# Diegotistical/OptionsLab

Hardware: AMD Instinct MI355X
Metric: MC path-steps/sec (1M paths × 252 steps Euro call); price vs BS |err|/σ (higher is better)
Workload: dtype f32 normals / f64 prices

## Files before the change

include/olmc.h:

```cpp
#ifndef OLMC_H
#define OLMC_H

#include <stdint.h>

#ifdef __cplusplus
extern "C" {
#endif

#define OLMC_ABI_VERSION 6

enum {
    OLMC_OK = 0,
    OLMC_ERR_ARG = 1,
    OLMC_ERR_HIP = 2,
    OLMC_ERR_STATE = 3,
    OLMC_ERR_RCCL = 4
};

enum { OLMC_STREAM_GBM = 0, OLMC_STREAM_HESTON = 1, OLMC_STREAM_JUMP = 2, OLMC_STREAM_KOU = 3 };
enum { OLMC_STREAM_HESTON_QE = 0x48514500 };
enum { OLMC_AVG_ARITHMETIC = 0, OLMC_AVG_GEOMETRIC = 1, OLMC_AVG_ARITHMETIC_FAST = 2 };
#define OLMC_MAX_BATCH 16

typedef struct olmc_stats {
// ... 269 lines not shown
                               int n_gpus, olmc_cv_moments* out);
int olmc_multi_gpu_european_qmc(double S, double K, double T, double r, double sigma, double q, int is_call,
                                int64_t n_paths, int32_t dims, const uint32_t* sv, const uint32_t* shift, int32_t bits,
                                int n_gpus, olmc_stats* out);
int olmc_multi_gpu_european_qmc_greeks_fd(double S, double K, double T, double r, double sigma, double q, int is_call,
                                          int64_t n_paths, int32_t dims, const uint32_t* sv, const uint32_t* shift, int32_t bits,
                                          int second_order, int n_gpus, double* out9, olmc_stats* evals );
int olmc_multi_gpu_european_qmc_cv(double S, double K, double T, double r, double sigma, double q, int is_call,
                                   int64_t n_paths, int32_t dims, const uint32_t* sv, const uint32_t* shift, int32_t bits,
                                   int n_gpus, olmc_cv_moments* out);
int olmc_multi_gpu_spans(double* out8);

int olmc_fetch_dev(const double* d_src, int32_t n, void* hip_stream, double* out_host);

int olmc_combine_stats(const olmc_stats* parts, int32_t n_parts, double r, double T, olmc_stats* out);

int olmc_philox_words(uint64_t seed, int64_t path_offset, int64_t n_paths,
                      int32_t block0, int32_t n_blocks, uint32_t stream_tag, uint32_t* out_host);
int olmc_normals(uint64_t seed, int64_t path_offset, int64_t n_paths, int32_t n_steps,
                 float* out_host);

int olmc_profile_enable(int on);
enum { OLMC_TUNE_GRID_CAP = 2, OLMC_TUNE_QMC_BLOCK = 4, OLMC_TUNE_SPLIT_TAIL = 7, OLMC_TUNE_POLL = 8, OLMC_TUNE_SPLIT_SAT = 9,
       OLMC_TUNE_MULTI_LAUNCH = 10, OLMC_TUNE_STAGED_COPY = 11, OLMC_TUNE_PHILOX_TABLE = 12 };
int olmc_tune(int knob, int value);
int olmc_profile_reset(void);
int olmc_kernel_time(int64_t* launches, double* total_ms);

#ifdef __cplusplus
}
#endif
#endif
```

include/olmc_probe.h:

```cpp
#ifndef OLMC_PROBE_H
#define OLMC_PROBE_H
#include "olmc.h"

#ifdef __cplusplus
extern "C" {
#endif

int olmc_exp2_probe(const double* x_host, int64_t n, double* y_host);
int olmc_exp2_probe_form(const double* x_host, int64_t n, double* y_host, int form);
int olmc_ndtri_probe(const double* p_host, int64_t n, double* z_host, int form);
int olmc_box_muller_probe(const uint32_t* xa, const uint32_t* xb, int64_t n, float* z_cos, float* z_sin, float* pair);
int olmc_sqrt_nonneg_probe(const double* x, int64_t n, double* y);
int olmc_normal_moments(uint64_t seed, int64_t path_offset, int64_t n_paths, int32_t n_steps, double* out4);
int olmc_reduce_probe(int nv, int form, int values, int blocking, int32_t launches, const int64_t* n_threads, const uint64_t* salt,
                      double* out);
int olmc_rows_sum_probe(int nv, int whole_workgroup, const double* rows_host, int32_t rows, double* out_nv);
int olmc_wave_reduce_probe(int p, int op, const double* v_host, double* out);

int olmc_phase_stamps(int64_t n_paths, int32_t n_steps, uint64_t seed, int32_t lead_launches, uint64_t* stamps_host, int64_t capacity,
                      int64_t* info3);

int olmc_clock_probe(int64_t n_paths, int32_t n_steps, uint64_t seed, double* out3);

enum { OLMC_PROBE_MAD_U64_U32 = 0, OLMC_PROBE_BITOP3_B32, OLMC_PROBE_CVT_F32_U32, OLMC_PROBE_FMAMK_F32, OLMC_PROBE_AND_OR_B32,
       OLMC_PROBE_LOG_F32, OLMC_PROBE_SQRT_F32, OLMC_PROBE_SIN_F32, OLMC_PROBE_COS_F32, OLMC_PROBE_EXP_F32, OLMC_PROBE_ADD_F32,
       OLMC_PROBE_FMA_F32, OLMC_PROBE_CVT_F64_F32, OLMC_PROBE_ADD_F64, OLMC_PROBE_FMA_F64, OLMC_PROBE_RNDNE_F64,
       OLMC_PROBE_LDEXP_F64, OLMC_PROBE_CVT_I32_F64,
       OLMC_PROBE_MIX_LOG_ADD, OLMC_PROBE_MIX_LOG_BITOP3, OLMC_PROBE_BITOP3_VVV, OLMC_PROBE_BITOP3_VVC, OLMC_PROBE_XOR_VV,
       OLMC_PROBE_MIX_BITOP3_ADD, OLMC_PROBE_MIX_MAD_BITOP3, OLMC_PROBE_MAD_U64_U32_VV, OLMC_PROBE_COUNT };
int olmc_issue_probe(int op, int waves_per_simd, double* ns_per_instr);

int olmc_european_f64_normals(double S, double K, double T, double r, double sigma, double q, int is_call, int64_t n_paths,
                              int32_t n_steps, uint64_t seed, olmc_stats* out);

int olmc_launch_gap_probe(int32_t n, double* us_per_launch);

enum { OLMC_PROBE_TUNE_FAULT_SHARD = 5, OLMC_PROBE_TUNE_FORCE_NV = 6, OLMC_PROBE_TUNE_MULTI_REHEARSAL = 11, OLMC_PROBE_TUNE_EXPECT_TABLE = 12 };
int olmc_probe_tune(int knob, int value);

#ifdef __cplusplus
}
#endif
#endif
```

optionslab_amd/_hip.py:

```python
from __future__ import annotations

import ctypes as C
import importlib.util
import os
import sys
import threading
from typing import List, Optional, Sequence, Tuple

import numpy as np

from .exceptions import AccelerationError

LIBRARY_PATH = os.environ.get("OLMC_LIBRARY") or os.path.join(os.path.dirname(os.path.abspath(__file__)), "libolmc.so")
MAX_BATCH = 16
AVG_ARITHMETIC, AVG_GEOMETRIC, AVG_ARITHMETIC_FAST = 0, 1, 2
_U64 = (1 << 64) - 1


class Stats(C.Structure):
    _fields_ = [("sum", C.c_double), ("sumsq", C.c_double), ("n", C.c_int64),
                ("price", C.c_double), ("std_error", C.c_double)]


class Option(C.Structure):
# ... 964 lines not shown


def philox_words(seed: int, path_offset: int, n_paths: int, block0: int, n_blocks: int, tag: int = 0) -> np.ndarray:
    out = np.empty((int(n_paths), int(n_blocks), 4), dtype=np.uint32)
    _check(lib().olmc_philox_words(seed64(seed), int(path_offset), int(n_paths), int(block0), int(n_blocks), int(tag),
                                   _pointer(out, C.c_uint32)))
    return out


def normals(seed: int, path_offset: int, n_paths: int, n_steps: int) -> np.ndarray:
    out = np.empty((int(n_paths), int(n_steps)), dtype=np.float32)
    _check(lib().olmc_normals(seed64(seed), int(path_offset), int(n_paths), int(n_steps), _pointer(out, C.c_float)))
    return out


TUNE_GRID_CAP = 2
TUNE_QMC_BLOCK = 4
TUNE_SPLIT_TAIL = 7
TUNE_POLL = 8
TUNE_SPLIT_SAT = 9
TUNE_MULTI_LAUNCH = 10
TUNE_STAGED_COPY = 11
TUNE_PHILOX_TABLE = 12


def tune(knob: int, value: int) -> None:
    _check(load_library().olmc_tune(int(knob), int(value)))


def profile_enable(on: bool) -> None:
    _check(lib().olmc_profile_enable(int(on)))


def profile_reset() -> None:
    _check(lib().olmc_profile_reset())


def kernel_time() -> Tuple[int, float]:
    n, ms = C.c_int64(0), C.c_double(0.0)
    _check(lib().olmc_kernel_time(C.byref(n), C.byref(ms)))
    return n.value, ms.value
```

optionslab_amd/csrc/olmc.hip:

```cpp
#include "olmc.h"
#include "olmc_local_vol.h"
#include "olmc_local_vol_qmc.h"
#include "olmc_jump.h"
#include "olmc_kernels.h"
#include "olmc_local_vol_kernels.h"
#include "olmc_local_vol_qmc_kernels.h"
#include "olmc_jump_kernels.h"
#include "olmc_jump_scenario_kernels.h"
#include "olmc_job_board.h"
#include "olmc_device_mem.h"

#include <dlfcn.h>
#include <sched.h>
#include <time.h>
#include <hip/hip_ext.h>
#include <rccl/rccl.h>

#include <algorithm>
#include <atomic>
#include <chrono>
#include <climits>
#include <condition_variable>
#include <cmath>
#include <cstdio>
// ... 47 lines not shown
    int device = -1;
    int cus = 0;
    hipStream_t stream = nullptr;
    struct WsSlot {
        DeviceBlock<Mem> block_rows;
        DeviceBlock<Mem> group_rows;
        DeviceBlock<Mem> counters;
        hipEvent_t done = nullptr;
        bool used = false;
        bool claimed = false;
        hipStream_t owner = nullptr;
        bool shared = false;
    };
    static constexpr int kSlots = 8;
    WsSlot slots[kSlots + 1];
    int next_slot = 0, cur_slot = 0;
    uint64_t* h_flag = nullptr;
    uint64_t* d_flag = nullptr;
    uint64_t seq = 0;
    uint64_t armed = 0;
    PinnedBlock<Mem> result;
    double* h_result = nullptr;
    double* d_result = nullptr;
    DeviceBlock<Mem> bulk;
    PinnedBlock<Mem> stage[2];
    hipEvent_t stage_landed[2] = {nullptr, nullptr};
    BatchWorkspace<Mem, MultiOption, kMultiCounterStride> multi;
    CachedUpload<Mem> sobol;
    CachedUpload<Mem> bridge;
    DeviceBlock<Mem> heston_w;
    CachedUpload<Mem> lv;
    int drain() const { return Mem::wait(stream); }
    bool busy = false;
    std::vector<EventPair> ev_free, ev_pending;
    int64_t prof_launches = 0;
    double prof_ms = 0.0;
};

constexpr int kMaxContexts = 8;

struct DevicePool {
    std::mutex mu;
    std::condition_variable idle;
    std::vector<DeviceCtx*> all;
    int device = -1;
};
// ... 1 lines not shown
std::mutex g_mu;
std::atomic<DevicePool*> g_pool[kMaxDevices] = {};
std::atomic<int> g_default_device{-1};
bool g_profile = false;

int no_users() { return 0; }

int ctx_allocate(DeviceCtx* c) {
    HIP_TRY(hipStreamCreateWithFlags(&c->stream, hipStreamNonBlocking));
    for (auto& sl : c->slots) {
        int rc = sl.group_rows.reserve(sizeof(double) * kMaxNV * kMaxGroups, no_users);
        if (!rc) rc = sl.counters.reserve(kCounterBytes, no_users);
        if (rc) return rc;
        HIP_TRY(hipMemset(sl.counters.get(), 0, kCounterBytes));
        HIP_TRY(hipEventCreateWithFlags(&sl.done, hipEventDisableTiming));
    }
    const int rc = c->result.reserve(sizeof(double) * (kMaxNV + 1 + 15), no_users, 0, 0, true);
    if (rc) return rc;
    c->h_result = c->result.as<double>();
    c->d_result = c->result.alias<double>();
    c->h_flag = reinterpret_cast<uint64_t*>(c->h_result + kMaxNV + 8);
    c->d_flag = reinterpret_cast<uint64_t*>(c->d_result + kMaxNV + 8);
    *c->h_flag = 0;
    return OLMC_OK;
}

void ctx_release(DeviceCtx* c) {
    if (c->stream) (void)hipStreamSynchronize(c->stream);
    for (auto& ep : c->ev_pending) { (void)hipEventDestroy(ep.start); (void)hipEventDestroy(ep.stop); }
    for (auto& ep : c->ev_free) { (void)hipEventDestroy(ep.start); (void)hipEventDestroy(ep.stop); }
    for (hipEvent_t ev : c->stage_landed)
        if (ev) (void)hipEventDestroy(ev);
    for (auto& sl : c->slots)
        if (sl.done) (void)hipEventDestroy(sl.done);
    if (c->stream) (void)hipStreamDestroy(c->stream);
    delete c;
}

int ctx_create(int device, DeviceCtx** out) {
    int count = 0;
    hipError_t e = hipGetDeviceCount(&count);
    if (e != hipSuccess || count <= 0)
        return fail(OLMC_ERR_HIP, std::string("no HIP device available: ") + hipGetErrorString(e));
    if (device < 0 || device >= count || device >= kMaxDevices)
        return fail(OLMC_ERR_ARG, "device index out of range");
    HIP_TRY(hipSetDevice(device));
// ... 12 lines not shown
}

struct CtxLease {
    DeviceCtx* c = nullptr;
    DevicePool* pool = nullptr;
    CtxLease() = default;
    CtxLease(const CtxLease&) = delete;
    CtxLease& operator=(const CtxLease&) = delete;
    ~CtxLease() { release(); }
    void release() {
        if (!c) return;
        {
            std::lock_guard<std::mutex> lock(pool->mu);
            c->busy = false;
        }
        pool->idle.notify_all();
        c = nullptr;
    }
};

int ctx_lease_on(int dev, CtxLease* out) {
    DevicePool* pool = g_pool[dev].load(std::memory_order_acquire);
    if (!pool) return fail(OLMC_ERR_STATE, "device not initialised (call olmc_init)");
    HIP_TRY(hipSetDevice(dev));
    std::unique_lock<std::mutex> lock(pool->mu);
    for (;;) {
        for (DeviceCtx* c : pool->all)
            if (!c->busy) {
                c->busy = true;
                out->c = c;
                out->pool = pool;
                return OLMC_OK;
            }
        if (static_cast<int>(pool->all.size()) < kMaxContexts) {
            DeviceCtx* c = nullptr;
            const int rc = ctx_create(dev, &c);
            if (rc) return rc;
            c->busy = true;
            pool->all.push_back(c);
            out->c = c;
            out->pool = pool;
            return OLMC_OK;
        }
        pool->idle.wait(lock);
    }
}

// ... 91 lines not shown
    }
    if (err == hipSuccess) landed.store(n_chunks, std::memory_order_release);
    else give_up.store(true);
    const auto t_join = clock::now();
    for (std::thread& t : threads) t.join();
    if (trace)
        std::fprintf(stderr, "[olmc copy_to_host] %.1f MB, %lld chunks, %d threads: spawn %.0f us, first chunk landed (kernel + DMA) %.0f us, later event waits %.0f us, "
                             "waits for the copy threads %.0f us, last chunk out + join %.0f us, total %.0f us\n", bytes / 1e6, static_cast<long long>(n_chunks), n_threads,
                     us_spawn, us_first, us_events, us_workers, us_since(t_join), us_since(t_begin));
    if (err != hipSuccess) {
        (void)hipStreamSynchronize(c->stream);
        (void)hipGetLastError();
        return fail(OLMC_ERR_HIP, std::string("copy_to_host: ") + hipGetErrorString(err));
    }
    return OLMC_OK;
}

int g_multi_launch = 0;
int g_grid_cap = 0;
int g_qmc_block = 0;
int g_poll = 0;
int g_split_tail = 0;
int g_philox_table = 1;
int g_split_sat = 0;
#ifdef OLMC_WITH_PROBES
int g_fault_shard = 0;
int g_force_nv = 0;
int g_multi_rehearsal = 0;
int g_expect_table = 0;
std::atomic<int> g_expect_table_misses{0};
#endif

int32_t grid_for(int64_t n_paths, int32_t n_steps = INT32_MAX) { return path_grid(n_paths, n_steps, g_grid_cap); }

template <typename Kernel>
int resident_workgroups(Kernel kernel) {
    static std::mutex mu;
    static std::vector<std::pair<const void*, int>> cache;
    const void* key = reinterpret_cast<const void*>(kernel);
    std::lock_guard<std::mutex> lock(mu);
    for (const auto& e : cache)
        if (e.first == key) return e.second;
    int nb = 0;
    if (hipOccupancyMaxActiveBlocksPerMultiprocessor(&nb, kernel, kBlock, 0) != hipSuccess || nb < 1) {
        (void)hipGetLastError();
        nb = 1;
    }
    cache.emplace_back(key, nb);
    return nb;
}

int32_t european_launch_shape(const DeviceCtx* c, PathRange* pr, int occ, bool keep_grid = false) {
// ... 3 lines not shown
    const int64_t wgs = (pr->count + kBlock - 1) / kBlock;
    if (g_split_tail < 0 || grid_cap != 0 || wgs != grid) return grid;
    if ((pr->n_steps >> 2) / kGroup < 4 || c->cus < 1) return grid;
    int64_t per_cu = (pr->count / kBlock) / c->cus;
    if (occ >= 1 && g_split_sat > 0) {
        const int64_t r = per_cu % occ;
        if (r > 0 && r < std::min(g_split_sat, occ)) per_cu -= r;
    }
    const int64_t full = per_cu * c->cus;
    const int64_t rest = pr->count - full * kBlock;
    if (rest == 0) return grid;
    const int64_t split = (rest + kWave - 1) / kWave;
    if (full + split > kMaxGrid) return grid;
    pr->split_from = static_cast<int32_t>(full);
    return static_cast<int32_t>(full + split);
}

template <int NSETS, int MODE>
int european_occupancy(bool anti) {
    if (g_split_sat <= 0) return 0;
    return anti ? resident_workgroups(european_path_kernel<NSETS, true, MODE, false>) : resident_workgroups(european_path_kernel<NSETS, false, MODE, false>);
}

int make_ws(DeviceCtx* c, hipStream_t stream, int32_t grid, int nv, double* d_out, double tail, ReduceWs* ws) {
    const bool own = stream == c->stream;
    int idx = DeviceCtx::kSlots;
    if (!own) {
        idx = -1;
        for (int i = 0; i < DeviceCtx::kSlots && idx < 0; ++i)
            if (c->slots[i].claimed && !c->slots[i].shared && c->slots[i].owner == stream) idx = i;
        for (int i = 0; i < DeviceCtx::kSlots && idx < 0; ++i)
            if (!c->slots[i].claimed) { c->slots[i].claimed = true; c->slots[i].owner = stream; idx = i; }
        if (idx < 0) {
            idx = c->next_slot;
            c->next_slot = (c->next_slot + 1) % DeviceCtx::kSlots;
            DeviceCtx::WsSlot& taken = c->slots[idx];
            if (!taken.shared) {
                HIP_TRY(hipDeviceSynchronize());
                taken.shared = true;
                taken.used = false;
            }
        }
    }
    DeviceCtx::WsSlot& sl = c->slots[idx];
    c->cur_slot = idx;
    const bool guarded = !own && sl.shared;
    const size_t need = static_cast<size_t>(grid) * nv;
    int rc = sl.block_rows.reserve(sizeof(double) * need, [&] {
        if (!guarded) HIP_TRY(hipStreamSynchronize(stream));
        else if (sl.used) HIP_TRY(hipEventSynchronize(sl.done));
        return static_cast<int>(OLMC_OK);
    }, sizeof(double) << 16);
    if (rc) return rc;
    if (guarded && sl.used) HIP_TRY(hipStreamWaitEvent(stream, sl.done, 0));
    ws->block_rows = sl.block_rows.as<double>();
    ws->group_rows = sl.group_rows.as<double>();
    ws->counters = sl.counters.as<uint32_t>();
    ws->out = d_out;
    ws->tail = tail;
    ws->row_capacity = sl.block_rows.capacity() / sizeof(double);
#ifdef OLMC_WITH_PROBES
    if (g_force_nv > 0) ws->row_capacity = static_cast<uint64_t>(grid) * g_force_nv;
#endif
    ws->done_flag = nullptr;
    ws->done_value = 0;
    c->armed = 0;
    if (own && d_out == c->d_result && g_poll >= 0) {
        c->armed = ++c->seq;
        ws->done_flag = c->d_flag;
        ws->done_value = c->armed;
    }
    return OLMC_OK;
}

void ws_recover(DeviceCtx* c) {
    c->armed = 0;
    (void)hipDeviceSynchronize();
    (void)hipGetLastError();
    for (auto& sl : c->slots) (void)hipMemset(sl.counters.get(), 0, kCounterBytes);
}

void multi_recover(DeviceCtx* c) {
    c->armed = 0;
    (void)hipDeviceSynchronize();
    (void)hipGetLastError();
    if (c->multi.counters()) (void)hipMemset(c->multi.counters(), 0, c->multi.counter_bytes());
}

int after_launch(DeviceCtx* c, hipStream_t stream) {
    hipError_t e = hipGetLastError();
    if (e != hipSuccess) { ws_recover(c); return fail(OLMC_ERR_HIP, std::string("kernel launch: ") + hipGetErrorString(e)); }
    if (c->cur_slot == DeviceCtx::kSlots || !c->slots[c->cur_slot].shared) return OLMC_OK;
    DeviceCtx::WsSlot& sl = c->slots[c->cur_slot];
    HIP_TRY(hipEventRecord(sl.done, stream));
    sl.used = true;
    return OLMC_OK;
}

int prof_begin(DeviceCtx* c, hipStream_t s, EventPair* ep) {
    if (c->ev_free.empty()) {
        HIP_TRY(hipEventCreate(&ep->start));
        HIP_TRY(hipEventCreate(&ep->stop));
    } else {
        *ep = c->ev_free.back();
        c->ev_free.pop_back();
    }
// ... 172 lines not shown
            launch_european<1, kReduce>(anti, g, st, pr, cs, ws, nullptr, timed);
        } else if (nsets == 8) {
            fused(std::integral_constant<int, 8>{});
        } else {
            fused(std::integral_constant<int, 16>{});
        }
    }, profiled);
}

constexpr int64_t kSpinUs = 200, kYieldUs = 2000, kSleepUs = 20;

struct TimerSlack {
    long old = -1;
    void tighten() {
        if (old >= 0) return;
        old = prctl(PR_GET_TIMERSLACK, 0, 0, 0, 0);
        if (old >= 0 && prctl(PR_SET_TIMERSLACK, 1000UL, 0, 0, 0) != 0) old = -1;
    }
    ~TimerSlack() {
        if (old >= 0) (void)prctl(PR_SET_TIMERSLACK, static_cast<unsigned long>(old), 0, 0, 0);
    }
};

int wait_armed(DeviceCtx* c, hipStream_t s) {
    if (c->armed != 0) {
        const uint64_t want = c->armed;
        c->armed = 0;
        using clock = std::chrono::steady_clock;
        const auto t0 = clock::now();
        bool queried = false;
        int phase = 0;
        TimerSlack slack;
        for (uint32_t spins = 0;; ++spins) {
            if (__atomic_load_n(c->h_flag, __ATOMIC_ACQUIRE) == want) {
                if (queried) (void)hipGetLastError();
                return OLMC_OK;
            }
            if (phase == 0) {
                __builtin_ia32_pause();
                if ((spins & 0x3F) == 0x3F && clock::now() - t0 >= std::chrono::microseconds(kSpinUs)) phase = 1;
                continue;
            }
            if (phase == 1) {
                sched_yield();
                if ((spins & 0xF) == 0xF && clock::now() - t0 >= std::chrono::microseconds(kYieldUs)) phase = 2;
                continue;
            }
            if ((spins & 0x3F) == 0) {
                const hipError_t q = hipStreamQuery(s);
                queried = true;
                if (q == hipSuccess) break;
                if (q != hipErrorNotReady) {
                    ws_recover(c);
                    return fail(OLMC_ERR_HIP, std::string("hipStreamQuery: ") + hipGetErrorString(q));
                }
            }
            slack.tighten();
            const timespec nap{0, kSleepUs * 1000};
            nanosleep(&nap, nullptr);
        }
        (void)hipGetLastError();
    }
    hipError_t e = hipStreamSynchronize(s);
    if (e != hipSuccess) { ws_recover(c); return fail(OLMC_ERR_HIP, std::string("hipStreamSynchronize: ") + hipGetErrorString(e)); }
    return OLMC_OK;
}

int sync_or_recover(DeviceCtx* c, hipStream_t s) {
    if (s != c->stream) c->armed = 0;
    return wait_armed(c, s);
}

int run_batch(const olmc_option* opts, int32_t k, int64_t path_offset, int64_t n_local, int32_t n_steps,
              uint64_t seed, int antithetic, olmc_stats* out, bool prices_only = false, bool keep_grid = false) {
    if (!opts || !out) return fail(OLMC_ERR_ARG, "null pointer");
    if (k < 1 || k > OLMC_MAX_BATCH) return fail(OLMC_ERR_ARG, "batch size must be in [1, OLMC_MAX_BATCH]");
    int rc = check_paths(path_offset, n_local, n_steps);
    if (rc) return rc;
    CtxLease lease;
    rc = ctx_lease(&lease);
    if (rc) return rc;
    DeviceCtx* const c = lease.c;
    int pos[OLMC_MAX_BATCH];
    bool lean = prices_only;
    rc = run_batch_device(c, c->stream, opts, k, path_offset, n_local, n_steps, seed, antithetic, c->d_result, -1.0, pos, true, &lean, keep_grid);
    if (rc) return rc;
    finish_set(c->h_result, pos, n_local * (antithetic ? 2 : 1), opts, k, false, lean, out);
    return OLMC_OK;
}

}

// ... 91 lines not shown
                                       int64_t path_offset, int64_t n_local, int32_t n_steps, uint64_t seed,
                                       int antithetic, double* d_triple, void* hip_stream) {
    if (!d_triple) return fail(OLMC_ERR_ARG, "null pointer");
    int rc = check_paths(path_offset, n_local, n_steps);
    if (rc) return rc;
    CtxLease lease;
    rc = ctx_lease(&lease);
    if (rc) return rc;
    DeviceCtx* const c = lease.c;
    hipStream_t s = static_cast<hipStream_t>(hip_stream);
    const olmc_option o = make_option(S, K, T, r, sigma, q, is_call);
    const double n = static_cast<double>(n_local * (antithetic ? 2 : 1));
    return run_batch_device(c, s, &o, 1, path_offset, n_local, n_steps, seed, antithetic, d_triple, n, nullptr, true);
}

namespace {
int fetch_dev(DeviceCtx* c, const double* d_src, int32_t n, hipStream_t s, double* out_host) {
    const uint64_t want = ++c->seq;
    hipLaunchKernelGGL(publish_kernel, dim3(1), dim3(kWave), 0, s, d_src, n, c->d_result, c->d_flag, want);
    HIP_TRY(hipGetLastError());
    int rc = OLMC_OK;
    if (g_poll >= 0) {
        c->armed = want;
        rc = wait_armed(c, s);
    } else {
        hipError_t e = hipStreamSynchronize(s);
        if (e != hipSuccess) rc = fail(OLMC_ERR_HIP, std::string("hipStreamSynchronize: ") + hipGetErrorString(e));
    }
    if (rc) return rc;
    for (int32_t i = 0; i < n; ++i) out_host[i] = c->h_result[i];
    return OLMC_OK;
}
}

extern "C" int olmc_fetch_dev(const double* d_src, int32_t n, void* hip_stream, double* out_host) {
    if (!d_src || !out_host) return fail(OLMC_ERR_ARG, "null pointer");
    if (n < 1 || n > kMaxNV + 1) return fail(OLMC_ERR_ARG, "n must be in [1, 33]");
    CtxLease lease;
    int rc = ctx_lease(&lease);
    if (rc) return rc;
    return fetch_dev(lease.c, d_src, n, static_cast<hipStream_t>(hip_stream), out_host);
}

extern "C" int olmc_european_batch(const olmc_option* opts, int32_t k, int64_t path_offset, int64_t n_local,
                                   int32_t n_steps, uint64_t seed, int antithetic, olmc_stats* out) {
    return run_batch(opts, k, path_offset, n_local, n_steps, seed, antithetic, out);
// ... 14 lines not shown
    if (rc) return rc;
    CtxLease lease;
    rc = ctx_lease(&lease);
    if (rc) return rc;
    DeviceCtx* const c = lease.c;
    const int32_t bpo = static_cast<int32_t>(std::min<int64_t>((n_paths + kBlock - 1) / kBlock, 1024));
    decltype(c->multi)::Views v;
    rc = c->multi.reserve(static_cast<size_t>(n_options), static_cast<size_t>(bpo), c->stream, &v);
    if (rc) return rc;
    MultiOption* const h = v.h_opts;
    for (int64_t j = 0; j < n_options; ++j) {
        const Contract ct = make_contract(opts[j], n_steps);
        h[j].a = ct.a; h[j].vol = ct.vol; h[j].strike = ct.strike; h[j].sign = ct.sign;
        h[j].tag = tags ? tags[j] : static_cast<uint32_t>(j);
        h[j].pad = 0;
    }
    HIP_TRY(hipMemcpyAsync(v.d_opts, h, sizeof(MultiOption) * n_options, hipMemcpyHostToDevice, c->stream));
    MultiDone md;
    md.done_count = v.d_done;
    md.n_total = static_cast<uint32_t>(n_options);
    md.done_flag = nullptr;
    md.done_value = 0;
    c->armed = 0;
    if (g_poll >= 0) {
        c->armed = ++c->seq;
        md.done_flag = c->d_flag;
        md.done_value = c->armed;
    }
    const PathRange pr = make_range(0, n_paths, n_steps, seed);
    EventPair ep{};
    if (g_profile) { rc = prof_begin(c, c->stream, &ep); if (rc) return rc; }
    for (int64_t base_opt = 0; base_opt < n_options; base_opt += 65535) {
        const unsigned ny = static_cast<unsigned>(std::min<int64_t>(65535, n_options - base_opt));
        with_bool(antithetic != 0, [&](auto a) { launch_timed(european_multi_kernel<a>, dim3(bpo, ny), dim3(kBlock), c->stream, nullptr, pr, v.d_opts, base_opt, v.d_rows, v.d_cnt, v.d_out, md); });
        hipError_t e = hipGetLastError();
        if (e != hipSuccess) {
            multi_recover(c);
            return fail(OLMC_ERR_HIP, std::string("kernel launch: ") + hipGetErrorString(e));
        }
    }
    if (g_profile) { rc = prof_end(c, c->stream, ep); if (rc) { multi_recover(c); return rc; } }
    rc = wait_armed(c, c->stream);
    if (rc) { multi_recover(c); return rc; }
    finish_set(v.h_out, nullptr, n_paths * (antithetic ? 2 : 1), opts, n_options, false, false, out);
    return OLMC_OK;
}
// ... 2745 lines not shown
    Carver bulk;
    rc = bulk_reserve(c, bytes, &bulk);
    if (rc) return rc;
    float* d_z = bulk.take<float>(bytes / sizeof(float));
    const int64_t total = n_paths * ((n_steps + 3) / 4);
    const int grid = static_cast<int>(std::min<int64_t>((total + 255) / 256, 4096));
    hipLaunchKernelGGL(normals_kernel, dim3(grid), dim3(256), 0, c->stream, static_cast<uint64_t>(path_offset), n_paths,
                       n_steps, static_cast<uint32_t>(seed), static_cast<uint32_t>(seed >> 32), d_z);
    HIP_TRY(hipGetLastError());
    HIP_TRY(hipMemcpyAsync(out_host, d_z, bytes, hipMemcpyDeviceToHost, c->stream));
    HIP_TRY(hipStreamSynchronize(c->stream));
    return OLMC_OK;
}

extern "C" int olmc_tune(int knob, int value) {
    if (knob == OLMC_TUNE_GRID_CAP && value >= 0) { g_grid_cap = value; return OLMC_OK; }
    if (knob == OLMC_TUNE_QMC_BLOCK && value >= -1 && value <= 2) { g_qmc_block = value; return OLMC_OK; }
    if (knob == OLMC_TUNE_POLL && value >= -1 && value <= 0) { g_poll = value; return OLMC_OK; }
    if (knob == OLMC_TUNE_SPLIT_TAIL && value >= -1 && value <= 0) { g_split_tail = value; return OLMC_OK; }
    if (knob == OLMC_TUNE_SPLIT_SAT && value >= 0 && value <= 16) { g_split_sat = value; return OLMC_OK; }
    if (knob == OLMC_TUNE_MULTI_LAUNCH && value >= -1 && value <= 0) { g_multi_launch = value; return OLMC_OK; }
    if (knob == OLMC_TUNE_STAGED_COPY && value >= -1 && value <= 0) { g_staged_copy = value; return OLMC_OK; }
    if (knob == OLMC_TUNE_PHILOX_TABLE && value >= 0 && value <= 1) { g_philox_table = value; return OLMC_OK; }
    return fail(OLMC_ERR_ARG, "unknown tuning knob or value");
}

namespace {
template <typename Fn>
int with_all_contexts(Fn fn) {
    int dev = t_device >= 0 ? t_device : g_default_device.load(std::memory_order_acquire);
    if (dev < 0) {
        int rc = olmc_init(0);
        if (rc) return rc;
        dev = t_device;
    }
    DevicePool* pool = g_pool[dev].load(std::memory_order_acquire);
    if (!pool) return fail(OLMC_ERR_STATE, "device not initialised (call olmc_init)");
    HIP_TRY(hipSetDevice(dev));
    std::vector<DeviceCtx*> mine;
    {
        std::unique_lock<std::mutex> lock(pool->mu);
        pool->idle.wait(lock, [&] { return std::none_of(pool->all.begin(), pool->all.end(), [](const DeviceCtx* c) { return c->busy; }); });
        mine = pool->all;
        for (DeviceCtx* c : mine) c->busy = true;
    }
    int rc = OLMC_OK;
// ... 56 lines not shown
```

optionslab_amd/csrc/olmc_host_math.h:

```cpp
#ifndef OLMC_HOST_MATH_H
#define OLMC_HOST_MATH_H

#include "olmc.h"
#include "olmc_jump_scenarios.h"

#include <algorithm>
#include <cmath>
#include <cstdint>
#include <cstring>

namespace olmc {

struct Contract {
    double a;
    double vol;
    double strike;
    double sign;
    double scale;
    double neg_sign_strike;
    double sign_scale;
};

template <int NSETS>
struct ContractSet {
// ... 581 lines not shown
    sh.blocks = qmc_block == 1 ? true : (qmc_block != 0 ? false : n_paths >= (int64_t(1) << blocks_from_log2));
    const int64_t split_grid = (n_paths + kWave - 1) / kWave;
    sh.split = !sh.blocks && (qmc_block == 0 || qmc_block == 2) && dims >= 16 && split_grid <= kMaxGrid;
    sh.units = sh.blocks ? (point_offset + n_paths + kQmcBlock - 1) / kQmcBlock - point_offset / kQmcBlock : n_paths;
    sh.grid = sh.split ? static_cast<int32_t>(split_grid) : path_grid(sh.units, INT32_MAX, grid_cap);
    return sh;
}

struct HestonSlabs {
    size_t slab;
    int32_t fit;
    int32_t grid;
    size_t bytes;
};
inline HestonSlabs heston_slab_shape(int32_t n_steps, int32_t grid, int cus, int32_t factors = 2) {
    HestonSlabs s;
    s.slab = static_cast<size_t>(factors) * static_cast<size_t>(n_steps) * kWave * sizeof(double);
    s.fit = static_cast<int32_t>(std::max<size_t>(kHestonSlabCap / (s.slab * kWavesPerBlock), 1));
    s.grid = std::min(grid, std::min(s.fit, std::max(cus, 1) * kHestonBridgeBlocksPerCu));
    s.bytes = s.slab * kWavesPerBlock * static_cast<size_t>(s.grid);
    return s;
}

}

#endif
```

optionslab_amd/csrc/olmc_kernels.h:

```cpp
#pragma once
#include <type_traits>
#include <hip/hip_runtime.h>
#include <stdint.h>

#include "olmc_host_math.h"

namespace olmc {



struct Words4 {
    uint32_t x0, x1, x2, x3;
};

__device__ __forceinline__ uint32_t xor3(uint32_t a, uint32_t b, uint32_t c) {
    return __builtin_amdgcn_bitop3_b32(a, b, c, 0x96);
}

__device__ __forceinline__ Words4 philox4x32_10(uint32_t c0, uint32_t c1, uint32_t c2, uint32_t c3,
                                                uint32_t k0, uint32_t k1) {
#pragma unroll
    for (int round = 0; round < 10; ++round) {
        const uint64_t p0 = static_cast<uint64_t>(kPhiloxM0) * c0;
        const uint64_t p1 = static_cast<uint64_t>(kPhiloxM1) * c2;
// ... 163 lines not shown
                                                  uint32_t tag = 0u) {
    return path_normal_quarters(g_lo, g_hi, n_steps, 0, 4, k0, k1, tag) * kPairZScale;
}

__device__ __forceinline__ double wave_sum(double v) {
#pragma unroll
    for (int off = kWave / 2; off > 0; off >>= 1) v += __shfl_down(v, off, kWave);
    return v;
}

constexpr int kGroupBlocks = 256;
constexpr int kGroupRowsCapacity = ((1 << 18) / kGroupBlocks + 1) * 32;
constexpr int kCounterStride = 64;

struct ReduceWs {
    double* block_rows;
    double* group_rows;
    uint32_t* counters;
    double* out;
    double tail;
    uint64_t row_capacity;
    uint64_t* done_flag;
    uint64_t done_value;
};

__device__ __forceinline__ void signal_done(const ReduceWs& ws) {
    if (ws.done_flag == nullptr) return;
    __builtin_amdgcn_fence(__ATOMIC_RELEASE, "");
    if (threadIdx.x == 0) __hip_atomic_store(ws.done_flag, ws.done_value, __ATOMIC_RELAXED, __HIP_MEMORY_SCOPE_SYSTEM);
}

#ifndef OLMC_AGENT_ACQUIRE
#define OLMC_AGENT_ACQUIRE 1
#endif
#if !OLMC_AGENT_ACQUIRE && defined(__HIP_DEVICE_COMPILE__) && !defined(__gfx942__) && !defined(__gfx950__)
#error "OLMC_AGENT_ACQUIRE=0 relies on gfx942 / gfx950 cache behaviour (sc1 rows are L2-served): build this target with the acquire"
#endif
__device__ __forceinline__ void acquire_rows() {
#if OLMC_AGENT_ACQUIRE
    __builtin_amdgcn_fence(__ATOMIC_ACQUIRE, "agent");
#else
    __builtin_amdgcn_fence(__ATOMIC_ACQUIRE, "wavefront");
#endif
}

__device__ __forceinline__ void store_sc1(double* p, double v) {
    __hip_atomic_store(p, v, __ATOMIC_RELAXED, __HIP_MEMORY_SCOPE_AGENT);
// ... 11 lines not shown
    double v = 0.0;
    if (c < NV) {
        constexpr int kBatch = 8;
        for (int32_t row = sub; row < rows; row += SUBS * kBatch) {
            double t[kBatch];
#pragma unroll
            for (int j = 0; j < kBatch; ++j) {
                const int32_t rj = row + j * SUBS;
                t[j] = rj < rows ? load_sc1(src + static_cast<size_t>(rj) * NV + c) : 0.0;
            }
#pragma unroll
            for (int j = 0; j < kBatch; ++j) v += t[j];
        }
    }
#pragma unroll
    for (int off = kWave / 2; off >= NVP; off >>= 1) v += __shfl_down(v, off, kWave);
    return v;
}

struct NoEpilogue {
    __device__ __forceinline__ void operator()(double) const {}
};

template <int NV, typename Epilogue = NoEpilogue>
__device__ __forceinline__ void grid_reduce(double v, const ReduceWs& ws, Epilogue done = Epilogue()) {
    const int lane = threadIdx.x;
    const int32_t n_blocks = static_cast<int32_t>(gridDim.x);
    const int32_t n_groups = (n_blocks + kGroupBlocks - 1) / kGroupBlocks;
    const int32_t group = static_cast<int32_t>(blockIdx.x) / kGroupBlocks;
    const int32_t group_size = min(kGroupBlocks, n_blocks - group * kGroupBlocks);

    if (static_cast<uint64_t>(n_blocks) * NV > ws.row_capacity || n_groups * NV > kGroupRowsCapacity) {
        if (blockIdx.x == 0) {
            if (lane < NV) ws.out[lane] = __builtin_nan("");
            signal_done(ws);
        }
        return;
    }
    if (lane < NV) store_sc1(ws.block_rows + static_cast<size_t>(blockIdx.x) * NV + lane, v);
    asm volatile("s_waitcnt vmcnt(0)" ::: "memory");
    uint32_t ticket = 0;
    if (lane == 0) ticket = __hip_atomic_fetch_add(ws.counters + static_cast<size_t>(group) * kCounterStride, 1u, __ATOMIC_RELAXED, __HIP_MEMORY_SCOPE_AGENT);
    ticket = __builtin_amdgcn_readfirstlane(ticket);
    if (ticket != static_cast<uint32_t>(group_size - 1)) return;

    acquire_rows();
    const double g = wave_rows_sum<NV>(ws.block_rows + static_cast<size_t>(group) * kGroupBlocks * NV, group_size);
    if (n_groups == 1) {
        if (lane < NV) ws.out[lane] = g;
        if (lane == 0) {
            if (ws.tail >= 0.0) ws.out[NV] = ws.tail;
            __hip_atomic_store(ws.counters, 0u, __ATOMIC_RELAXED, __HIP_MEMORY_SCOPE_AGENT);
        }
        done(g);
        signal_done(ws);
        return;
    }
    if (lane < NV) store_sc1(ws.group_rows + static_cast<size_t>(group) * NV + lane, g);
    asm volatile("s_waitcnt vmcnt(0)" ::: "memory");
    if (lane == 0) {
        __hip_atomic_store(ws.counters + static_cast<size_t>(group) * kCounterStride, 0u, __ATOMIC_RELAXED, __HIP_MEMORY_SCOPE_AGENT);
        ticket = __hip_atomic_fetch_add(ws.counters + static_cast<size_t>(n_groups) * kCounterStride, 1u, __ATOMIC_RELAXED, __HIP_MEMORY_SCOPE_AGENT);
    }
    ticket = __builtin_amdgcn_readfirstlane(ticket);
    if (ticket != static_cast<uint32_t>(n_groups - 1)) return;

    acquire_rows();
    const double total = wave_rows_sum<NV>(ws.group_rows, n_groups);
    if (lane < NV) ws.out[lane] = total;
    if (lane == 0) {
// ... 14 lines not shown
        constexpr int kBatch = NVP >= 16 ? 16 : 8;
        for (int32_t row = sub; row < rows; row += SUBS * kBatch) {
            double t[kBatch];
#pragma unroll
            for (int j = 0; j < kBatch; ++j) {
                const int32_t rj = row + j * SUBS;
                t[j] = rj < rows ? load_sc1(src + static_cast<size_t>(rj) * NV + c) : 0.0;
            }
#pragma unroll
            for (int j = 0; j < kBatch; ++j) v += t[j];
        }
    }
    part[threadIdx.x] = v;
    __syncthreads();
    double total = 0.0;
    if (threadIdx.x < NV) {
#pragma unroll
        for (int k = 0; k < SUBS; ++k) total += part[k * NVP + threadIdx.x];
    }
    __syncthreads();
    return total;
}

template <int NV, typename Epilogue = NoEpilogue>
__device__ __forceinline__ void grid_reduce_workgroup(double v, const ReduceWs& ws, Epilogue done = Epilogue()) {
    __shared__ double part[kBlock];
    __shared__ uint32_t last;
    const int t = threadIdx.x;
    const bool wave0 = t < kWave;
    const int32_t n_blocks = static_cast<int32_t>(gridDim.x);
    const int32_t n_groups = (n_blocks + kGroupBlocks - 1) / kGroupBlocks;
    const int32_t group = static_cast<int32_t>(blockIdx.x) / kGroupBlocks;
    const int32_t group_size = min(kGroupBlocks, n_blocks - group * kGroupBlocks);

    if (static_cast<uint64_t>(n_blocks) * NV > ws.row_capacity || n_groups * NV > kGroupRowsCapacity) {
        if (blockIdx.x == 0 && wave0) {
            if (t < NV) ws.out[t] = __builtin_nan("");
            signal_done(ws);
        }
        return;
    }
    if (wave0) {
        if (t < NV) store_sc1(ws.block_rows + static_cast<size_t>(blockIdx.x) * NV + t, v);
        asm volatile("s_waitcnt vmcnt(0)" ::: "memory");
        if (t == 0) last = __hip_atomic_fetch_add(ws.counters + static_cast<size_t>(group) * kCounterStride, 1u, __ATOMIC_RELAXED, __HIP_MEMORY_SCOPE_AGENT) ==
                           static_cast<uint32_t>(group_size - 1);
    }
    __syncthreads();
    if (!last) return;

    acquire_rows();
    const double g = workgroup_rows_sum<NV>(ws.block_rows + static_cast<size_t>(group) * kGroupBlocks * NV, group_size, part);
    if (n_groups == 1) {
        if (wave0) {
            if (t < NV) ws.out[t] = g;
            if (t == 0) {
                if (ws.tail >= 0.0) ws.out[NV] = ws.tail;
                __hip_atomic_store(ws.counters, 0u, __ATOMIC_RELAXED, __HIP_MEMORY_SCOPE_AGENT);
            }
            done(g);
            signal_done(ws);
        }
        return;
    }
    if (wave0) {
        if (t < NV) store_sc1(ws.group_rows + static_cast<size_t>(group) * NV + t, g);
        asm volatile("s_waitcnt vmcnt(0)" ::: "memory");
        if (t == 0) {
            __hip_atomic_store(ws.counters + static_cast<size_t>(group) * kCounterStride, 0u, __ATOMIC_RELAXED, __HIP_MEMORY_SCOPE_AGENT);
            last = __hip_atomic_fetch_add(ws.counters + static_cast<size_t>(n_groups) * kCounterStride, 1u, __ATOMIC_RELAXED, __HIP_MEMORY_SCOPE_AGENT) ==
                   static_cast<uint32_t>(n_groups - 1);
        }
    }
    __syncthreads();
    if (!last) return;
// ... 3577 lines not shown
```

Baseline: 2518 billion.

## Publish per-group sums as tagged pinned records and finish reduction on host

Instead of a second device-side stage (last group reduces all group rows and then signals a done flag), each group's last block writes its sum into pinned host memory as a self-validating record (value plus value XOR a sequence tag). The host poller collects all the records and sums them in the device's order. This removes the cross-group atomic ticket and final reduction from the kernel tail, shortening the critical path before completion is visible. It also skips hipSetDevice when the device is already current. The cost is a more complex host poll loop, reliance on 128-bit write atomicity to pinned memory, and an extra fallback path when records are not all seen.

```diff
diff --git a/include/olmc.h b/include/olmc.h
--- a/include/olmc.h
+++ b/include/olmc.h
@@ -315,7 +315,7 @@
 
 int olmc_profile_enable(int on);
 enum { OLMC_TUNE_GRID_CAP = 2, OLMC_TUNE_QMC_BLOCK = 4, OLMC_TUNE_SPLIT_TAIL = 7, OLMC_TUNE_POLL = 8, OLMC_TUNE_SPLIT_SAT = 9,
-       OLMC_TUNE_MULTI_LAUNCH = 10, OLMC_TUNE_STAGED_COPY = 11, OLMC_TUNE_PHILOX_TABLE = 12 };
+       OLMC_TUNE_MULTI_LAUNCH = 10, OLMC_TUNE_STAGED_COPY = 11, OLMC_TUNE_PHILOX_TABLE = 12, OLMC_TUNE_RECORDS = 13 };
 int olmc_tune(int knob, int value);
 int olmc_profile_reset(void);
 int olmc_kernel_time(int64_t* launches, double* total_ms);
diff --git a/include/olmc_probe.h b/include/olmc_probe.h
--- a/include/olmc_probe.h
+++ b/include/olmc_probe.h
@@ -35,7 +35,9 @@
 
 int olmc_launch_gap_probe(int32_t n, double* us_per_launch);
 
-enum { OLMC_PROBE_TUNE_FAULT_SHARD = 5, OLMC_PROBE_TUNE_FORCE_NV = 6, OLMC_PROBE_TUNE_MULTI_REHEARSAL = 11, OLMC_PROBE_TUNE_EXPECT_TABLE = 12 };
+enum { OLMC_PROBE_TUNE_FAULT_SHARD = 5, OLMC_PROBE_TUNE_FORCE_NV = 6, OLMC_PROBE_TUNE_MULTI_REHEARSAL = 11, OLMC_PROBE_TUNE_EXPECT_TABLE = 12,
+       OLMC_PROBE_TUNE_STAMP_RECORDS = 13,
+       OLMC_PROBE_TUNE_RECORD_LAUNCHES = 14 };
 int olmc_probe_tune(int knob, int value);
 
 #ifdef __cplusplus
diff --git a/optionslab_amd/_hip.py b/optionslab_amd/_hip.py
--- a/optionslab_amd/_hip.py
+++ b/optionslab_amd/_hip.py
@@ -1010,6 +1010,7 @@
 TUNE_MULTI_LAUNCH = 10
 TUNE_STAGED_COPY = 11
 TUNE_PHILOX_TABLE = 12
+TUNE_RECORDS = 13
 
 
 def tune(knob: int, value: int) -> None:
diff --git a/optionslab_amd/csrc/olmc.hip b/optionslab_amd/csrc/olmc.hip
--- a/optionslab_amd/csrc/olmc.hip
+++ b/optionslab_amd/csrc/olmc.hip
@@ -93,6 +93,11 @@
     PinnedBlock<Mem> result;
     double* h_result = nullptr;
     double* d_result = nullptr;
+    PinnedBlock<Mem> records;
+    uint64_t* h_records = nullptr;
+    uint64_t* d_records = nullptr;
+    int32_t rec_groups = 0;
+    int rec_nv = 0;
     DeviceBlock<Mem> bulk;
     PinnedBlock<Mem> stage[2];
     hipEvent_t stage_landed[2] = {nullptr, nullptr};
@@ -140,6 +145,11 @@
     c->h_flag = reinterpret_cast<uint64_t*>(c->h_result + kMaxNV + 8);
     c->d_flag = reinterpret_cast<uint64_t*>(c->d_result + kMaxNV + 8);
     *c->h_flag = 0;
+    const int rc_rec = c->records.reserve(sizeof(uint64_t) * 2 * kRecordSlots, no_users, 0, 0, true);
+    if (rc_rec) return rc_rec;
+    c->h_records = c->records.as<uint64_t>();
+    c->d_records = c->records.alias<uint64_t>();
+    std::memset(c->h_records, 0, sizeof(uint64_t) * 2 * kRecordSlots);
     return OLMC_OK;
 }
 
@@ -198,7 +208,8 @@
 int ctx_lease_on(int dev, CtxLease* out) {
     DevicePool* pool = g_pool[dev].load(std::memory_order_acquire);
     if (!pool) return fail(OLMC_ERR_STATE, "device not initialised (call olmc_init)");
-    HIP_TRY(hipSetDevice(dev));
+    int current = -1;
+    if (hipGetDevice(&current) != hipSuccess || current != dev) HIP_TRY(hipSetDevice(dev));
     std::unique_lock<std::mutex> lock(pool->mu);
     for (;;) {
         for (DeviceCtx* c : pool->all)
@@ -336,12 +347,15 @@
 int g_poll = 0;
 int g_split_tail = 0;
 int g_philox_table = 1;
+int g_records = 0;
 int g_split_sat = 0;
 #ifdef OLMC_WITH_PROBES
 int g_fault_shard = 0;
 int g_force_nv = 0;
 int g_multi_rehearsal = 0;
 int g_expect_table = 0;
+int g_stamp_records = 0;
+std::atomic<int64_t> g_record_launches{0};
 std::atomic<int> g_expect_table_misses{0};
 #endif
 
@@ -391,7 +405,9 @@
     return anti ? resident_workgroups(european_path_kernel<NSETS, true, MODE, false>) : resident_workgroups(european_path_kernel<NSETS, false, MODE, false>);
 }
 
-int make_ws(DeviceCtx* c, hipStream_t stream, int32_t grid, int nv, double* d_out, double tail, ReduceWs* ws) {
+constexpr int kRecordBound = kRecordSlots;
+
+int make_ws(DeviceCtx* c, hipStream_t stream, int32_t grid, int nv, double* d_out, double tail, ReduceWs* ws, bool allow_records = true) {
     const bool own = stream == c->stream;
     int idx = DeviceCtx::kSlots;
     if (!own) {
@@ -433,24 +449,46 @@
 #endif
     ws->done_flag = nullptr;
     ws->done_value = 0;
+    ws->records = nullptr;
+    ws->record_seq = 0;
     c->armed = 0;
+    c->rec_groups = 0;
     if (own && d_out == c->d_result && g_poll >= 0) {
         c->armed = ++c->seq;
-        ws->done_flag = c->d_flag;
-        ws->done_value = c->armed;
-    }
-    return OLMC_OK;
+        const int32_t n_groups = (grid + kGroupBlocks - 1) / kGroupBlocks;
+        const int64_t bound = g_records > 0 ? g_records : kRecordBound;
+        if (g_records >= 0 && allow_records && !(tail >= 0.0) && static_cast<int64_t>(n_groups) * nv <= bound) {
+            ws->records = c->d_records;
+#ifdef OLMC_WITH_PROBES
+            g_record_launches.fetch_add(1, std::memory_order_relaxed);
+#endif
+            ws->record_seq = record_tag(c->armed);
+            c->rec_groups = n_groups;
+            c->rec_nv = nv;
+        } else {
+            ws->done_flag = c->d_flag;
+            ws->done_value = c->armed;
+        }
+    }
+    return OLMC_OK;
+}
+
+int make_ws(DeviceCtx* c, hipStream_t stream, int32_t grid, int nv, double* d_out, double tail, HookedReduceWs* ws) {
+    return make_ws(c, stream, grid, nv, d_out, tail, static_cast<ReduceWs*>(ws), false);
 }
 
 void ws_recover(DeviceCtx* c) {
     c->armed = 0;
+    c->rec_groups = 0;
     (void)hipDeviceSynchronize();
     (void)hipGetLastError();
+    if (c->h_records) std::memset(c->h_records, 0, sizeof(uint64_t) * 2 * kRecordSlots);
     for (auto& sl : c->slots) (void)hipMemset(sl.counters.get(), 0, kCounterBytes);
 }
 
 void multi_recover(DeviceCtx* c) {
     c->armed = 0;
+    c->rec_groups = 0;
     (void)hipDeviceSynchronize();
     (void)hipGetLastError();
     if (c->multi.counters()) (void)hipMemset(c->multi.counters(), 0, c->multi.counter_bytes());
@@ -669,17 +707,30 @@
     }
 };
 
+bool take_records(DeviceCtx* c, uint64_t tag, int32_t n_groups, int nv, int32_t* next, double* sums) {
+    const int32_t n = n_groups * nv;
+    while (*next < n && record_take(c->h_records + 2 * static_cast<size_t>(*next), tag, &sums[*next])) ++*next;
+    if (*next < n) return false;
+    records_total(nv, sums, n_groups, c->h_result);
+    return true;
+}
+
 int wait_armed(DeviceCtx* c, hipStream_t s) {
     if (c->armed != 0) {
         const uint64_t want = c->armed;
         c->armed = 0;
+        const int32_t n_groups = c->rec_groups, n_records = n_groups * c->rec_nv;
+        c->rec_groups = 0;
+        const uint64_t tag = record_tag(want);
+        int32_t next_record = 0;
+        double sums[kRecordSlots];
         using clock = std::chrono::steady_clock;
         const auto t0 = clock::now();
         bool queried = false;
         int phase = 0;
         TimerSlack slack;
         for (uint32_t spins = 0;; ++spins) {
-            if (__atomic_load_n(c->h_flag, __ATOMIC_ACQUIRE) == want) {
+            if (n_records ? take_records(c, tag, n_groups, c->rec_nv, &next_record, sums) : __atomic_load_n(c->h_flag, __ATOMIC_ACQUIRE) == want) {
                 if (queried) (void)hipGetLastError();
                 return OLMC_OK;
             }
@@ -707,6 +758,13 @@
             nanosleep(&nap, nullptr);
         }
         (void)hipGetLastError();
+        if (n_records) {
+            hipError_t e = hipStreamSynchronize(s);
+            if (e != hipSuccess) { ws_recover(c); return fail(OLMC_ERR_HIP, std::string("hipStreamSynchronize: ") + hipGetErrorString(e)); }
+            if (take_records(c, tag, n_groups, c->rec_nv, &next_record, sums)) return OLMC_OK;
+            ws_recover(c);
+            return fail(OLMC_ERR_HIP, "a blocking launch retired without its group sums");
+        }
     }
     hipError_t e = hipStreamSynchronize(s);
     if (e != hipSuccess) { ws_recover(c); return fail(OLMC_ERR_HIP, std::string("hipStreamSynchronize: ") + hipGetErrorString(e)); }
@@ -715,6 +773,7 @@
 
 int sync_or_recover(DeviceCtx* c, hipStream_t s) {
     if (s != c->stream) c->armed = 0;
+    if (c->armed == 0) c->rec_groups = 0;
     return wait_armed(c, s);
 }
 
@@ -852,6 +911,7 @@
     int rc = OLMC_OK;
     if (g_poll >= 0) {
         c->armed = want;
+        c->rec_groups = 0;
         rc = wait_armed(c, s);
     } else {
         hipError_t e = hipStreamSynchronize(s);
@@ -912,6 +972,7 @@
     md.done_flag = nullptr;
     md.done_value = 0;
     c->armed = 0;
+    c->rec_groups = 0;
     if (g_poll >= 0) {
         c->armed = ++c->seq;
         md.done_flag = c->d_flag;
@@ -3703,6 +3764,7 @@
     if (knob == OLMC_TUNE_MULTI_LAUNCH && value >= -1 && value <= 0) { g_multi_launch = value; return OLMC_OK; }
     if (knob == OLMC_TUNE_STAGED_COPY && value >= -1 && value <= 0) { g_staged_copy = value; return OLMC_OK; }
     if (knob == OLMC_TUNE_PHILOX_TABLE && value >= 0 && value <= 1) { g_philox_table = value; return OLMC_OK; }
+    if (knob == OLMC_TUNE_RECORDS && value >= -1 && value <= kRecordSlots) { g_records = value; return OLMC_OK; }
     return fail(OLMC_ERR_ARG, "unknown tuning knob or value");
 }
 
diff --git a/optionslab_amd/csrc/olmc_host_math.h b/optionslab_amd/csrc/olmc_host_math.h
--- a/optionslab_amd/csrc/olmc_host_math.h
+++ b/optionslab_amd/csrc/olmc_host_math.h
@@ -627,6 +627,49 @@
     return s;
 }
 
+
+inline uint64_t record_tag(uint64_t seq) {
+    uint64_t z = seq + 0x9E3779B97F4A7C15ull;
+    z = (z ^ (z >> 30)) * 0xBF58476D1CE4E5B9ull;
+    z = (z ^ (z >> 27)) * 0x94D049BB133111EBull;
+    z ^= z >> 31;
+    return z ? z : 0x9E3779B97F4A7C15ull;
+}
+
+inline bool record_take(const uint64_t* rec, uint64_t tag, double* value) {
+    const uint64_t w0 = __atomic_load_n(rec, __ATOMIC_RELAXED), w1 = __atomic_load_n(rec + 1, __ATOMIC_RELAXED);
+    if ((w0 ^ w1) != tag) return false;
+    std::memcpy(value, &w0, sizeof(double));
+    return true;
+}
+
+inline void rows_sum_device_order(int nv, bool whole_workgroup, const double* src, int32_t rows, double* out) {
+    const int nvp = !whole_workgroup && nv <= 2 ? 2 : nv <= 8 ? 8 : nv <= 16 ? 16 : 32;
+    const int subs = (whole_workgroup ? kBlock : kWave) / nvp;
+    for (int c = 0; c < nv; ++c) {
+        double part[kBlock / 8];
+        for (int sub = 0; sub < subs; ++sub) {
+            double v = 0.0;
+            for (int32_t row = sub; row < rows; row += subs) v += src[static_cast<size_t>(row) * nv + c];
+            part[sub] = v;
+        }
+        if (whole_workgroup) {
+            double total = 0.0;
+            for (int k = 0; k < subs; ++k) total += part[k];
+            out[c] = total;
+        } else {
+            for (int d = subs / 2; d >= 1; d >>= 1)
+                for (int sub = 0; sub < d; ++sub) part[sub] += part[sub + d];
+            out[c] = part[0];
+        }
+    }
+}
+
+inline void records_total(int nv, const double* group_sums, int32_t n_groups, double* out) {
+    if (n_groups == 1) { for (int c = 0; c < nv; ++c) out[c] = group_sums[c]; return; }
+    rows_sum_device_order(nv, nv > 2, group_sums, n_groups, out);
+}
+
 }
 
 #endif
diff --git a/optionslab_amd/csrc/olmc_kernels.h b/optionslab_amd/csrc/olmc_kernels.h
--- a/optionslab_amd/csrc/olmc_kernels.h
+++ b/optionslab_amd/csrc/olmc_kernels.h
@@ -209,7 +209,22 @@
     uint64_t row_capacity;
     uint64_t* done_flag;
     uint64_t done_value;
-};
+    uint64_t* records;
+    uint64_t record_seq;
+};
+struct HookedReduceWs : ReduceWs {};
+
+constexpr int kRecordSlots = 1024;
+typedef unsigned long long RecordWords __attribute__((ext_vector_type(2)));
+
+template <int NV>
+__device__ __forceinline__ void write_record(const ReduceWs& ws, int32_t group, int c, double g) {
+    const int32_t slot = group * NV + c;
+    if (c >= NV || slot >= kRecordSlots) return;
+    const uint64_t bits = static_cast<uint64_t>(__double_as_longlong(g));
+    const RecordWords rec = {bits, bits ^ ws.record_seq};
+    *reinterpret_cast<volatile RecordWords*>(ws.records + 2 * slot) = rec;
+}
 
 __device__ __forceinline__ void signal_done(const ReduceWs& ws) {
     if (ws.done_flag == nullptr) return;
@@ -267,16 +282,31 @@
     __device__ __forceinline__ void operator()(double) const {}
 };
 
-template <int NV, typename Epilogue = NoEpilogue>
-__device__ __forceinline__ void grid_reduce(double v, const ReduceWs& ws, Epilogue done = Epilogue()) {
+template <typename Epilogue, typename Ws>
+__device__ __forceinline__ bool hands_records(const Ws& ws) {
+    static_assert(std::is_same<Epilogue, NoEpilogue>::value || std::is_same<Ws, HookedReduceWs>::value,
+                  "a kernel that passes an epilogue hook takes a HookedReduceWs (the make_ws overload that never arms records)");
+    if constexpr (std::is_same<Ws, HookedReduceWs>::value) return false;
+    else return ws.records != nullptr;
+}
+
+template <int NV>
+__device__ __forceinline__ void refuse_records(const ReduceWs& ws, int32_t n_groups) {
+    for (int32_t slot = threadIdx.x; slot < n_groups * NV && slot < kRecordSlots; slot += kWave) write_record<1>(ws, slot, 0, __builtin_nan(""));
+}
+
+template <int NV, typename Epilogue = NoEpilogue, typename Ws = ReduceWs>
+__device__ __forceinline__ void grid_reduce(double v, const Ws& ws, Epilogue done = Epilogue()) {
     const int lane = threadIdx.x;
     const int32_t n_blocks = static_cast<int32_t>(gridDim.x);
     const int32_t n_groups = (n_blocks + kGroupBlocks - 1) / kGroupBlocks;
     const int32_t group = static_cast<int32_t>(blockIdx.x) / kGroupBlocks;
     const int32_t group_size = min(kGroupBlocks, n_blocks - group * kGroupBlocks);
+    const bool records = hands_records<Epilogue, Ws>(ws);
 
     if (static_cast<uint64_t>(n_blocks) * NV > ws.row_capacity || n_groups * NV > kGroupRowsCapacity) {
         if (blockIdx.x == 0) {
+            if (records) { refuse_records<NV>(ws, n_groups); return; }
             if (lane < NV) ws.out[lane] = __builtin_nan("");
             signal_done(ws);
         }
@@ -291,6 +321,11 @@
 
     acquire_rows();
     const double g = wave_rows_sum<NV>(ws.block_rows + static_cast<size_t>(group) * kGroupBlocks * NV, group_size);
+    if (records) {
+        write_record<NV>(ws, group, lane, g);
+        if (lane == 0) __hip_atomic_store(ws.counters + static_cast<size_t>(group) * kCounterStride, 0u, __ATOMIC_RELAXED, __HIP_MEMORY_SCOPE_AGENT);
+        return;
+    }
     if (n_groups == 1) {
         if (lane < NV) ws.out[lane] = g;
         if (lane == 0) {
@@ -351,8 +386,8 @@
     return total;
 }
 
-template <int NV, typename Epilogue = NoEpilogue>
-__device__ __forceinline__ void grid_reduce_workgroup(double v, const ReduceWs& ws, Epilogue done = Epilogue()) {
+template <int NV, typename Epilogue = NoEpilogue, typename Ws = ReduceWs>
+__device__ __forceinline__ void grid_reduce_workgroup(double v, const Ws& ws, Epilogue done = Epilogue()) {
     __shared__ double part[kBlock];
     __shared__ uint32_t last;
     const int t = threadIdx.x;
@@ -361,9 +396,11 @@
     const int32_t n_groups = (n_blocks + kGroupBlocks - 1) / kGroupBlocks;
     const int32_t group = static_cast<int32_t>(blockIdx.x) / kGroupBlocks;
     const int32_t group_size = min(kGroupBlocks, n_blocks - group * kGroupBlocks);
+    const bool records = hands_records<Epilogue, Ws>(ws);
 
     if (static_cast<uint64_t>(n_blocks) * NV > ws.row_capacity || n_groups * NV > kGroupRowsCapacity) {
         if (blockIdx.x == 0 && wave0) {
+            if (records) { refuse_records<NV>(ws, n_groups); return; }
             if (t < NV) ws.out[t] = __builtin_nan("");
             signal_done(ws);
         }
@@ -380,6 +417,13 @@
 
     acquire_rows();
     const double g = workgroup_rows_sum<NV>(ws.block_rows + static_cast<size_t>(group) * kGroupBlocks * NV, group_size, part);
+    if (records) {
+        if (wave0) {
+            write_record<NV>(ws, group, t, g);
+            if (t == 0) __hip_atomic_store(ws.counters + static_cast<size_t>(group) * kCounterStride, 0u, __ATOMIC_RELAXED, __HIP_MEMORY_SCOPE_AGENT);
+        }
+        return;
+    }
     if (n_groups == 1) {
         if (wave0) {
             if (t < NV) ws.out[t] = g;
```

Measured after the change: 2548 billion, median of 6. About the same (+1.2%).
